# parsaeskandar/pangenome-index

Measured on AMD Instinct MI355X. Metric: find_mems reads/sec (150 bp batch), higher is better.
Workload: dtype u64

## Files before the change

### include/pgx.h

```cpp
#ifndef PGX_H
#define PGX_H

#include <stddef.h>
#include <stdint.h>

#ifdef __cplusplus
extern "C" {
#endif

#define PGX_ABI_VERSION 7

typedef enum {
    PGX_OK = 0,
    PGX_ERR_IO = 1,
    PGX_ERR_FORMAT = 2,
    PGX_ERR_UNSUPPORTED = 3,
    PGX_ERR_NO_DEVICE = 4,
    PGX_ERR_HIP = 5,
    PGX_ERR_ARG = 6,
    PGX_ERR_NOMEM = 7
} pgx_status;

#define PGX_MODE_COMPAT 0u
#define PGX_MODE_STRICT 1u
// ... 164 lines not shown
} pgx_timing;

#define PGX_KERNELS_FM 0x1u
#define PGX_KERNELS_FM_SEEDED 0x2u
#define PGX_KERNELS_FM_NARROW 0x4u
#define PGX_KERNELS_FM_KIND_SHIFT 3
#define PGX_KERNELS_FM_LDS 0x20u
#define PGX_KERNELS_FM_REDO 0x40u
#define PGX_KERNELS_PAIRS 0x100u
#define PGX_KERNELS_PAIRS_S64 0x200u
#define PGX_KERNELS_PAIRS_COOP 0x400u
#define PGX_KERNELS_PAIRS_PACKED 0x800u
#define PGX_KERNELS_PAIRS_WIDE 0x1000u
#define PGX_KERNELS_PAIRS_LCE 0x2000u
#define PGX_KERNELS_SIDE 0x10000u
#define PGX_KERNELS_HEAVY 0x20000u
#define PGX_KERNELS_FM_MASK 0x3Fu
#define PGX_KERNELS_PAIRS_MASK 0x3F00u
uint32_t pgx_kernel_variants(uint32_t *out, uint32_t cap);

pgx_status pgx_batch_create(pgx_index *h, int device, const uint8_t *reads, const uint64_t *offsets,
                            uint64_t n_reads, pgx_batch **out);
pgx_status pgx_host_alloc(size_t bytes, void **out);
void pgx_host_free(void *p);
pgx_status pgx_batch_upload(pgx_batch *b, const uint8_t *reads, const uint64_t *offsets, uint64_t n_reads);
pgx_status pgx_batch_upload_packed(pgx_batch *b, const uint32_t *packed, const uint64_t *offsets, uint64_t n_reads, const uint64_t *side_ids,
                                   const uint8_t *side_bytes, uint64_t n_side);
pgx_status pgx_pack_reads(const uint8_t *reads, const uint64_t *offsets, uint64_t n_reads, uint32_t threads, uint32_t *packed, uint64_t *side_ids,
                          uint64_t side_ids_cap, uint8_t *side_bytes, uint64_t side_bytes_cap, uint64_t *n_side, uint64_t *n_side_bytes);
#define PGX_READS_LINES 0u
// ... 76 lines not shown
```

### pangenome-index_amd/csrc/pgx_batch.hip

```cpp
#include <memory>
#include <string>
#include <thread>

#include "pgx_runtime_internal.hpp"

struct pgx_chunk { uint64_t r0, r1, slot_base, slots; };

struct pgx_batch {
    pgx_index *h = nullptr;
    pgx_device_image *dimg = nullptr;
    int device = 0;
    hipStream_t own = nullptr;
    hipStream_t side = nullptr;
    hipEvent_t ev_side[2] = {nullptr, nullptr};
    bool class_valid = false, class_ok = false;
    uint64_t side_reads_est = 0;
    uint64_t n_reads = 0, read_bytes = 0;
    HostBuf h_off[2];
    int h_off_cur = 0;
    const uint64_t *h_offsets() const { return h_off[h_off_cur].as<uint64_t>(); }
    std::vector<pgx_chunk> chunks;
    bool plan_valid = false, slot_off_valid = false;
    uint64_t slot_off_min_len = 0;
    uint64_t plan_min_len = 0, plan_budget = 0;
// ... 302 lines not shown
    return PGX_OK;
    PGX_GUARD_END
}


struct RunKnobs {
    bool spec;
    bool arena;
    bool has_arena_cap;
    uint64_t arena_cap;
    uint64_t budget_slots;
    bool narrow;
    bool force_redo;
    bool pairs;
    bool side;
    bool packed;
    int coop;
    bool lce;
    bool has_wg_per_cu;
    int wg_per_cu;
    uint32_t heavy_ext;
    bool has_side_heavy_ext;
    uint32_t side_heavy_ext;
    bool debug_counters;
    bool fm_stats;
};

static RunKnobs read_run_knobs() {
    auto is_set = [](const char *name) { return std::getenv(name) != nullptr; };
    auto not_zero = [](const char *name) { const char *e = std::getenv(name); return !(e && e[0] == '0'); };
    RunKnobs k{};
    k.spec = not_zero("PGX_SPEC");
    k.arena = not_zero("PGX_SLOT_ARENA");
    if (const char *e = std::getenv("PGX_SLOT_ARENA_CAP")) { k.has_arena_cap = true; k.arena_cap = std::strtoull(e, nullptr, 10); }
    if (const char *e = std::getenv("PGX_SLOT_BUDGET_MB")) k.budget_slots = std::max<uint64_t>(1, std::strtoull(e, nullptr, 10)) * (1ull << 20) / sizeof(pgx_mem);
    k.narrow = not_zero("PGX_FM_NARROW");
    k.force_redo = is_set("PGX_FM_NARROW_FORCE_REDO");
    k.pairs = not_zero("PGX_FM_PAIRS");
    k.side = !is_set("PGX_FM_NO_SIDE");
    k.packed = not_zero("PGX_FM_PACKED");
    k.coop = -1;
    if (const char *e = std::getenv("PGX_FM_COOP")) k.coop = e[0] == '1';
    k.lce = not_zero("PGX_FM_LCE");
    if (const char *e = std::getenv("PGX_FM_WG_PER_CU")) { k.has_wg_per_cu = true; k.wg_per_cu = std::atoi(e); }
    k.heavy_ext = PGX_FM_HEAVY_EXT;
    if (const char *e = std::getenv("PGX_FM_HEAVY_EXT")) k.heavy_ext = (uint32_t)std::strtoul(e, nullptr, 10);
    if (const char *e = std::getenv("PGX_FM_SIDE_HEAVY_EXT")) { k.has_side_heavy_ext = true; k.side_heavy_ext = (uint32_t)std::strtoul(e, nullptr, 10); }
    k.debug_counters = is_set("PGX_DEBUG_COUNTERS");
    k.fm_stats = is_set("PGX_FM_STATS");
    return k;
}

static const void *find_mems_entry(bool in_lds, uint32_t kind, bool narrow, bool seeded) {
    using K = const void *;
// ... 15 lines not shown
static uint32_t find_mems_bits(bool in_lds, uint32_t kind, bool narrow, bool seeded) {
    return PGX_KERNELS_FM | (seeded ? PGX_KERNELS_FM_SEEDED : 0u) | (narrow ? PGX_KERNELS_FM_NARROW : 0u) | (kind << PGX_KERNELS_FM_KIND_SHIFT) | (in_lds ? PGX_KERNELS_FM_LDS : 0u);
}

static const void *find_mems_variant(bool in_lds, uint32_t kind, bool narrow, bool seeded, uint32_t &bits) {
    if (kind == 0) seeded = false;
    const void *f = find_mems_entry(in_lds, kind, narrow, seeded);
    if (!f) throw Error(PGX_ERR_UNSUPPORTED, "pgx_batch_run: no find_mems kernel for this image");
    bits = find_mems_bits(in_lds, kind, narrow, seeded);
    return f;
}

static const void *find_mems_pairs_entry(bool wide, bool packed, bool coop, bool s64, bool lce) {
    using K = const void *;
    static const K plain[2][2] = {
        {(K)pgx_find_mems_pairs_kernel<true, false, false, false, false, false>, (K)pgx_find_mems_pairs_kernel<true, false, false, false, true, false>},
        {(K)pgx_find_mems_pairs_kernel<true, true, false, false, false, false>, (K)pgx_find_mems_pairs_kernel<true, true, false, false, true, false>}};
    static const K pack[2][2][2] = {
        {{(K)pgx_find_mems_pairs_kernel<true, false, true, false, false, false>, (K)pgx_find_mems_pairs_kernel<true, false, true, false, true, false>},
         {(K)pgx_find_mems_pairs_kernel<true, false, true, true, false, false>, (K)pgx_find_mems_pairs_kernel<true, false, true, true, true, false>}},
        {{(K)pgx_find_mems_pairs_kernel<true, true, true, false, false, false>, (K)pgx_find_mems_pairs_kernel<true, true, true, false, true, false>},
         {(K)pgx_find_mems_pairs_kernel<true, true, true, true, false, false>, (K)pgx_find_mems_pairs_kernel<true, true, true, true, true, false>}}};
    static const K with_lce[2] = {(K)pgx_find_mems_pairs_kernel<true, false, true, false, false, true>, (K)pgx_find_mems_pairs_kernel<true, false, true, false, true, true>};
    if (lce) return (wide || !packed || coop) ? nullptr : with_lce[s64];
    if (!packed) return coop ? nullptr : plain[wide][s64];
    return pack[wide][coop][s64];
}

static uint32_t find_mems_pairs_bits(bool wide, bool packed, bool coop, bool s64, bool lce) {
    return PGX_KERNELS_PAIRS | (s64 ? PGX_KERNELS_PAIRS_S64 : 0u) | (coop ? PGX_KERNELS_PAIRS_COOP : 0u) | (packed ? PGX_KERNELS_PAIRS_PACKED : 0u) |
           (wide ? PGX_KERNELS_PAIRS_WIDE : 0u) | (lce ? PGX_KERNELS_PAIRS_LCE : 0u);
}

static const void *find_mems_pairs_variant(bool wide, bool packed, bool coop, bool s64, bool lce, uint32_t &bits) {
    const void *f = find_mems_pairs_entry(wide, packed, coop, s64, lce);
    if (!f && lce) throw Error(PGX_ERR_UNSUPPORTED, "pgx_batch_run: no LCE pairs kernel for this image");
    if (!f) throw Error(PGX_ERR_UNSUPPORTED, "pgx_batch_run: no cooperative pairs kernel without the packed reads");
    bits = find_mems_pairs_bits(wide, packed, coop, s64, lce);
    return f;
}

// ... 11 lines not shown
    }
    return n;
}

struct RunCtx {
    pgx_batch *b;
    hipStream_t s;
    RunKnobs k;
    PgxDevImage img;
    uint64_t n, min_len, min_occ;
    bool want_tags;
    unsigned long long *ctr = nullptr;
    bool spec = false, arena_on = false;
    uint64_t cm_cap = 0;
    const void *kfn = nullptr, *kfn_wide = nullptr, *kfn_pairs = nullptr;
    uint32_t kfn_bits = 0, kfn_pairs_bits = 0;
    size_t pairs_lds = 0;
    int cus = 0;
    bool fresh_work = false, fresh_mark = false;
    uint64_t n_ext = 0;
    float ms_fm = 0, ms_cp = 0, ms_main = 0;
};

struct FmArgs {
    PgxDevImage img;
    const uint8_t *reads;
    const uint64_t *off, *slot_off;
    uint64_t n, min_len, min_occ, base, first;
    pgx_mem *slots;
    uint32_t *cnt;
// ... 62 lines not shown
    }
    uint64_t max_chunk_reads = 1;
    for (auto &c : b->chunks) max_chunk_reads = std::max(max_chunk_reads, c.r1 - c.r0);
    b->ovf_base.ensure(max_chunk_reads * 4);
}

static void choose_kernels(RunCtx &r) {
    pgx_batch *b = r.b;
    const PgxDevImage &img = r.img;
    const bool in_lds = b->dimg->lds_bytes != 0;
    const bool seeded = img.seed_k != 0 && r.min_len >= img.seed_k;
    r.kfn = r.kfn_wide = find_mems_variant(in_lds, img.dense, false, seeded, r.kfn_bits);
    bool c_fits = true;
    for (int i = 0; i < 8; i++) c_fits = c_fits && !(b->h->img.consts.C[i] >> 32);
    if (img.dense && img.dense != 3 && img.n < (1ull << 30) && c_fits && r.k.narrow) r.kfn = find_mems_variant(in_lds, img.dense, true, seeded, r.kfn_bits);
    r.kfn_pairs = nullptr;
    if (img.pairs && seeded && !(r.n >> 32) && b->read_bytes < (1ull << 35) && r.k.pairs)
        r.kfn_pairs = find_mems_pairs_variant(img.wide != 0, false, false, img.pairs_stride == PGX_PAIRS_STRIDE64, false, r.kfn_pairs_bits);
    r.pairs_lds = img.wide ? (size_t)img.n_sbp * 192 : 0;
    HIPCHECK(hipDeviceGetAttribute(&r.cus, hipDeviceAttributeMultiprocessorCount, b->device));
}

static void classify_reads(RunCtx &r, uint64_t cn) {
    pgx_batch *b = r.b;
    hipStream_t s = r.s;
    r.fresh_work = true;
    const uint64_t cap = std::max<uint64_t>(cn, 1024);
    b->read_flags.ensure(((cn + 3) & ~3ull) + 4);
    b->side_list.ensure((cn ? cn : 1) * sizeof(pgx_heavy_item));
    b->side_count.ensure(16);
    b->scan_tmp.ensure(cap * 8);
    b->scan_tmp.scan_epoch = 0;
    b->packed.ensure(((b->read_bytes + 15) / 16 + 64) * 4);
// ... 17 lines not shown
}

static void launch_side(RunCtx &r, FmArgs &a, const void *kf, unsigned grid) {
    pgx_batch *b = r.b;
    HIPCHECK(hipEventRecord(b->ev_side[0], r.s));
    HIPCHECK(hipStreamWaitEvent(b->side, b->ev_side[0], 0));
    const pgx_heavy_item *s_list = b->side_list.as<pgx_heavy_item>();
    const unsigned long long *s_count = b->side_count.as<unsigned long long>();
    unsigned long long *s_cur = r.ctr + PGX_CTR_SIDE_CURSOR;
    uint32_t s_hext = r.k.heavy_ext ? std::min<uint32_t>(r.k.heavy_ext, PGX_FM_SIDE_HEAVY_EXT) : 0u;
    if (r.k.has_side_heavy_ext) s_hext = r.k.side_heavy_ext;
    void *sargs[] = {&a.img, &a.reads, &a.off, &a.n, &a.min_len, &a.min_occ, &a.slot_off, &a.slots, &a.cnt, &a.next, &s_cur, &a.first, &a.base,
                     &s_hext, &a.hcap, &a.hlist, &a.hcount, &s_list, &s_count, &a.ovf, &a.ovf_cap};
    const uint64_t cus = (uint64_t)r.cus;
    const unsigned side_wgs = (unsigned)std::min<uint64_t>(4 * cus, std::max<uint64_t>(cus, b->side_reads_est / (2ull * PGX_FM_THREADS) + 1));
    HIPCHECK(hipLaunchKernel(kf, dim3(std::min<unsigned>(grid, side_wgs)), dim3(PGX_FM_THREADS), sargs, b->dimg->lds_bytes, b->side));
    b->timing.kernels |= r.kfn_bits | PGX_KERNELS_SIDE | (kf != r.kfn ? PGX_KERNELS_FM_REDO : 0u);
    HIPCHECK(hipEventRecord(b->ev_side[1], b->side));
}

static void launch_pairs(RunCtx &r, FmArgs &a, const uint8_t *skip, uint64_t cn, unsigned grid) {
    pgx_batch *b = r.b;
    const PgxDevImage &img = r.img;
    const void *kp = r.kfn_pairs;
    uint32_t kp_bits = r.kfn_pairs_bits;
    size_t plds = r.pairs_lds;
    const uint32_t *a_packed = nullptr;
    uint32_t a_pkw = 0;
    const uint32_t pkw = (uint32_t)((15 + b->max_read_len + 15) >> 4) + 1u;
    if (skip && pkw <= 24 && r.k.packed) {
        const bool coop = r.k.coop >= 0 ? r.k.coop != 0 : b->h->img.pairs.size() > (3ull << 30);
// ... 203 lines not shown
    pgx_batch *b = r.b;
    hipStream_t s = r.s;
    b->n_mems = b->n_positions = b->n_ext = b->n_tag_overflow = 0;
    std::memset(&b->timing, 0, sizeof b->timing);
    r.fresh_work = r.fresh_mark = false;
    r.n_ext = 0;
    r.ms_fm = r.ms_cp = r.ms_main = 0;
    b->counters.ensure(PGX_CTR_ALL * 8);
    HIPCHECK(hipMemsetAsync(b->counters.p, 0, PGX_CTR_ALL * 8, s));
    r.ctr = b->counters.as<unsigned long long>();

    record(b, 0, s);
    plan_slots(r);
    const std::vector<pgx_chunk> &chunks = b->chunks;
    r.arena_on = r.k.arena && !force_worst;
    r.kfn = r.kfn_wide = r.kfn_pairs = nullptr;
    r.cus = 0;
    if (r.n) choose_kernels(r);
    if (r.k.heavy_ext) {
        b->heavy_list.ensure((size_t)PGX_FM_HEAVY_CAP * sizeof(pgx_heavy_item));
        b->heavy_scratch.ensure((size_t)PGX_FM_HEAVY_GRID * PGX_FM_HEAVY_MAXLEN * sizeof(PgxHeavyResult));
    }
    r.spec = may_speculate && chunks.size() == 1 && b->shape_valid && b->shape_reads == r.n && b->shape_min_len == r.min_len && b->shape_min_occ == r.min_occ &&
             b->shape_tags == r.want_tags && (!r.want_tags || (b->tw.have_last && b->tw.last_largest <= PGX_SORT_WG_LDS_CAP)) && r.k.spec && !r.k.force_redo;
    r.cm_cap = with_slack(b->last_mems);
    uint64_t mem_base = 0;
    for (size_t ci = 0; ci < chunks.size(); ci++) {
        record(b, 1, s);
        uint64_t ovf_cap = 0;
        const uint64_t cm = find_mems_chunk(r, ci, ovf_cap);
        compact_chunk(r, chunks[ci], cm, mem_base, ovf_cap);
// ... 402 lines not shown
```

### pangenome-index_amd/csrc/pgx_device.h

```cpp
#pragma once

#include <hip/hip_runtime.h>
#include <stdint.h>

#include "../../include/pgx.h"
#include "pgx_image.h"

enum PgxCounterSlot {
    PGX_CTR_EXT = 0,
    PGX_CTR_TAG_OVERFLOW = 1,
    PGX_CTR_CURSOR = 5,
    PGX_CTR_HEAVY = 8,
    PGX_CTR_OVF32 = 9,
    PGX_CTR_MEMS = 10,
    PGX_CTR_REDO = 11,
    PGX_CTR_REDO_CURSOR = 12,
    PGX_CTR_SIDE_CURSOR = 13,
    PGX_CTR_OVF_TOP = 14,
    PGX_CTR_OVF_ABORT = 15,
    PGX_CTR_TAG0 = 16,
    PGX_CTR_ABORT = 30,
    PGX_CTR_PAIRS_LINES = 32,
    PGX_CTR_PAIRS_SEEDS = 33,
    PGX_CTR_FM_LINES = 34,
// ... 77 lines not shown
#define PGX_FM_HEAVY_GRID 64u
template <bool LDS_IMAGE>
__global__ void pgx_find_mems_heavy_kernel(PgxDevImage img, const uint8_t *reads, const uint64_t *offsets, uint64_t min_len, uint64_t min_occ,
                                           const uint64_t *slot_off, uint64_t slot_base, pgx_mem *slots, uint32_t *mem_count,
                                           unsigned long long *n_ext_total, const pgx_heavy_item *heavy_list,
                                           const unsigned long long *heavy_count, uint32_t heavy_cap, PgxHeavyResult *scratch, uint64_t chunk_first,
                                           uint64_t chunk_reads, uint32_t *ovf_base, uint64_t ovf_cap);

__global__ void pgx_seed_build_kernel(PgxDevImage img, const uint4 *src, uint4 *dst, uint32_t level, uint64_t n_dst, uint64_t limit, int end_table);
template <bool LDS_IMAGE, int DENSE, bool NARROW, bool SEED>
__global__ void pgx_find_mems_kernel(PgxDevImage img, const uint8_t *reads, const uint64_t *offsets, uint64_t n_reads,
                                     uint64_t min_len, uint64_t min_occ, const uint64_t *slot_off, pgx_mem *slots,
                                     uint32_t *mem_count, unsigned long long *n_ext_total, unsigned long long *cursor, uint64_t first_read,
                                     uint64_t slot_base, uint32_t heavy_ext, uint32_t heavy_cap, pgx_heavy_item *heavy_list, unsigned long long *heavy_count,
                                     const pgx_heavy_item *rid_list, const unsigned long long *rid_count, uint32_t *ovf_base, uint64_t ovf_cap);
template <bool SEED, bool WIDE, bool PACKED, bool COOP, bool S64, bool LCE>
__global__ void pgx_find_mems_pairs_kernel(PgxDevImage img, const uint8_t *reads, const uint64_t *offsets, uint64_t n_reads,
                                           uint64_t min_len, uint64_t min_occ, const uint64_t *slot_off, pgx_mem *slots,
                                           uint32_t *mem_count, unsigned long long *n_ext_total, unsigned long long *cursor, uint64_t first_read,
                                           uint64_t slot_base, uint32_t heavy_ext, uint32_t heavy_cap, pgx_heavy_item *heavy_list, unsigned long long *heavy_count,
                                           const uint8_t *skip, const uint32_t *packed, uint32_t pk_words,
                                           uint32_t *ovf_base, uint64_t ovf_cap);
__global__ void pgx_bad_chunks_kernel(const uint8_t *reads, uint64_t n_bytes, uint64_t *chunks, unsigned long long *count, uint64_t cap, uint32_t *packed);
__global__ void pgx_unpack_reads_kernel(const uint32_t *packed, uint64_t n_chunks, uint8_t *reads);
__global__ void pgx_side_reads_kernel(uint8_t *reads, const uint64_t *offsets, const uint64_t *side_ids, const uint64_t *side_off, const uint8_t *side_bytes, uint64_t n_side,
                                      uint8_t *flags, pgx_heavy_item *list, unsigned long long *count);
__global__ void pgx_classify_reads_kernel(const uint8_t *reads, const uint64_t *offsets, uint64_t n_reads, const uint64_t *chunks, const unsigned long long *n_chunks,
                                          uint64_t cap, uint32_t *flag_words, pgx_heavy_item *list, unsigned long long *count);
__global__ void pgx_first_ext_kernel(PgxDevImage img, uint4 *out);
__global__ void pgx_rank_kernel(PgxDevImage img, const uint64_t *pos, uint64_t n, int true_codes, uint64_t *out);
template <bool LOOP, bool MULHI> __global__ void pgx_rank_probe_kernel(PgxDevImage img, const uint64_t *pos, uint64_t n, uint64_t *out);
// ... 145 lines not shown
```

### pangenome-index_amd/csrc/pgx_kernels.hip

```cpp
#include <hip/hip_runtime.h>
#include <stdint.h>

#include <type_traits>

#include "pgx_device.h"

template <bool LDS_IMAGE>
__device__ __forceinline__ uint32_t pgx_find_block(const PgxDevImage &img, const uint64_t *__restrict__ lds_dir,
                                                   const uint16_t *__restrict__ lds_blow, uint64_t pos) {
    const uint64_t di = pos >> img.dir_shift;
    const uint64_t e = LDS_IMAGE ? lds_dir[di] : img.dir[di];
    const uint32_t lowp = (uint32_t)pos & ((1u << img.dir_shift) - 1u);
    uint32_t lo = (uint32_t)e;
    const uint32_t cnt = (uint32_t)(e >> 32) & 0xFFu;
    if (cnt <= 2) {
        const uint32_t l0 = (uint32_t)(e >> 40) & 0xFFFu, l1 = (uint32_t)(e >> 52);
        return lo - 1u + ((cnt >= 1 && l0 <= lowp) ? 1u : 0u) + ((cnt >= 2 && l1 <= lowp) ? 1u : 0u);
    }
    uint32_t hi = cnt < 255 ? lo + cnt : (uint32_t)(LDS_IMAGE ? lds_dir[di + 1] : img.dir[di + 1]);
    while (lo < hi) {
        const uint32_t mid = (lo + hi) >> 1;
        const uint32_t v = LDS_IMAGE ? lds_blow[mid] : img.blow[mid];
        if (v <= lowp) lo = mid + 1; else hi = mid;
    }
// ... 856 lines not shown
    if (k >= n_side) return;
    const uint64_t rid = side_ids[k], dst = offsets[rid], len = offsets[rid + 1] - dst, src = side_off[k];
    for (uint64_t i = lane; i < len; i += 64) reads[dst + i] = side_bytes[src + i];
    if (lane == 0) {
        flags[rid] = 1;
        pgx_heavy_item it;
        it.rid = rid; it.x = 0; it.nm = 0;
        list[k] = it;
        if (k == 0) *count = n_side;
    }
}

__device__ __forceinline__ uint32_t pgx_window_byte(uint64_t w0, uint64_t w1, uint64_t a) {
    return (uint32_t)(((a & 8ull) ? w1 : w0) >> (8u * (uint32_t)(a & 7ull))) & 0xFFu;
}
template <bool SEED, bool WIDE, bool PACKED, bool COOP, bool S64, bool LCE>
#ifndef PGX_LCE_WAVES
#define PGX_LCE_WAVES PGX_FM_WAVES_PER_SIMD
#endif
__global__ void __launch_bounds__(PGX_FM_THREADS, LCE ? PGX_LCE_WAVES : ((PACKED && !WIDE && !COOP) ? PGX_PAIRS_PACKED_WAVES : PGX_FM_WAVES_PER_SIMD))
pgx_find_mems_pairs_kernel(PgxDevImage img, const uint8_t *__restrict__ reads, const uint64_t *__restrict__ offsets,
                           uint64_t n_reads, uint64_t min_len, uint64_t min_occ, const uint64_t *__restrict__ slot_off,
                           pgx_mem *__restrict__ slots, uint32_t *__restrict__ mem_count, unsigned long long *__restrict__ n_ext_total,
                           unsigned long long *__restrict__ cursor, uint64_t first_read, uint64_t slot_base, uint32_t heavy_ext, uint32_t heavy_cap,
                           pgx_heavy_item *__restrict__ heavy_list, unsigned long long *__restrict__ heavy_count, const uint8_t *__restrict__ skip,
                           const uint32_t *__restrict__ packed, uint32_t pk_words, uint32_t *__restrict__ ovf_base, uint64_t ovf_cap) {
    typedef typename std::conditional<WIDE, uint64_t, uint32_t>::type pos_t;
    __shared__ uint32_t s_ext[512];
    __shared__ pos_t s_C[8];
    __shared__ pos_t s_t2[32];
    __shared__ uint4 s_fe[PACKED ? 16 : 512];
    extern __shared__ __align__(16) unsigned char pgx_dyn_lds[];
    static_assert(!COOP || PACKED, "the cooperative loads come with the packed reads");
    static_assert(!LCE || (PACKED && !WIDE && !COOP), "the text comparison reads the packed reads and 32-bit suffix array entries");
    constexpr uint32_t SYMS = PGX_PAIRS_SYMS, STRIDE = S64 ? PGX_PAIRS_STRIDE64 : PGX_PAIRS_SYMS;
    uint32_t *s_rd = reinterpret_cast<uint32_t *>(pgx_dyn_lds);
    const uint32_t rd_stride = blockDim.x;
    uint4 *s_stage = reinterpret_cast<uint4 *>(pgx_dyn_lds + (size_t)pk_words * PGX_FM_THREADS * 4) + (size_t)(threadIdx.x >> 6) * 512;
    uint64_t *s_pb = reinterpret_cast<uint64_t *>(pgx_dyn_lds + (size_t)pk_words * PGX_FM_THREADS * 4 + (COOP ? (size_t)(PGX_FM_THREADS / 64) * 8192 : 0));
    uint4 *s_sa4 = reinterpret_cast<uint4 *>(pgx_dyn_lds + (size_t)pk_words * PGX_FM_THREADS * 4);
    uint32_t *s_sae = reinterpret_cast<uint32_t *>(s_sa4 + PGX_FM_THREADS);
    uint32_t *s_lcp = s_sae + PGX_FM_THREADS;
    for (uint32_t i = threadIdx.x; i < 512; i += blockDim.x) s_ext[i] = img.consts->ext_tab[i];
    if (threadIdx.x < 8) s_C[threadIdx.x] = (pos_t)img.consts->C[threadIdx.x];
    if (threadIdx.x < 32) s_t2[threadIdx.x] = (pos_t)img.consts->pair_t2w[threadIdx.x];
    if (WIDE) for (uint32_t i = threadIdx.x; i < img.n_sbp * 24u; i += blockDim.x) s_pb[i] = img.pbase[i];
    if (PACKED) { if (threadIdx.x < 9) s_fe[threadIdx.x] = img.first_ext[threadIdx.x == 4 ? 0u : (threadIdx.x > 4 ? 256u : 0u) + ((0x47544341u >> (8u * ((threadIdx.x > 4 ? threadIdx.x - 5u : threadIdx.x) & 3u))) & 0xFFu)]; }
    else for (uint32_t i = threadIdx.x; i < 512; i += blockDim.x) s_fe[i] = img.first_ext[i];
    __syncthreads();
// ... 88 lines not shown
        restart = more ? restart : 1u;
    };

    for (;;) {
        __builtin_amdgcn_s_setprio(3);
        unsigned long long idle = __ballot(ph == 0);
        if (LCE && idle && (uint32_t)__popcll(idle) < img.refill_min && __popcll(idle) != 64) idle = 0ull;
#ifdef PGX_FM_STATS
        const unsigned long long st_r0 = __builtin_readcyclecounter();
        if (idle) st_refills++;
#endif
        while (idle) {
            if (rnext == rend) {
                if (exhausted) break;
                unsigned long long got = 0;
                if (lane == 0) got = first_read + atomicAdd(cursor, 32ull);
                got = ((unsigned long long)(uint32_t)__builtin_amdgcn_readfirstlane((int)(uint32_t)(got >> 32)) << 32) |
                      (uint32_t)__builtin_amdgcn_readfirstlane((int)(uint32_t)got);
                if (got >= n_reads) { exhausted = true; break; }
                rnext = got;
                rend = got + 32ull < n_reads ? got + 32ull : n_reads;
            }
            const uint64_t avail = rend - rnext;
            const uint32_t rank = (uint32_t)__popcll(idle & ((1ull << lane) - 1ull));
            if (ph == 0 && (uint64_t)rank < avail) {
                rid = (uint32_t)(rnext + rank);
                const uint8_t *skp = skip ? skip + rid : reinterpret_cast<const uint8_t *>(offsets);
                const uint32_t skv = (uint32_t)*skp;
                const uint64_t o0 = offsets[rid], o1 = offsets[rid + 1];
                const uint32_t sk = skip ? skv : 0u;
                base = o0;
                len = (int32_t)(o1 - o0);
                if (sk) ph = -1;
                else {
                    if (PACKED) {
                        const uint32_t *src = packed + (base >> 4);
                        const uint32_t nw = ((uint32_t)(base & 15ull) + (uint32_t)len + 15u) >> 4;
#pragma unroll 1
                        for (uint32_t w0 = 0; w0 < nw; w0 += PGX_PK_GROUP) {
                            uint32_t t[PGX_PK_GROUP];
#pragma unroll
                            for (uint32_t i = 0; i < PGX_PK_GROUP; i++) t[i] = src[w0 + i < nw ? w0 + i : nw - 1u];
#pragma unroll
                            for (uint32_t i = 0; i < PGX_PK_GROUP; i++) if (w0 + i < nw) s_rd[(w0 + i) * rd_stride + threadIdx.x] = t[i];
                        }
                    }
                    x = 0; nm = 0;
                    next0 = next;
                    begin();
                    if (ph == 0) ph = -1;
                }
            }
            const uint32_t want = (uint32_t)__popcll(idle);
            rnext += (uint64_t)want < avail ? (uint64_t)want : avail;
            idle = __ballot(ph == 0);
        }
#ifdef PGX_FM_STATS
        asm volatile("s_waitcnt vmcnt(0) lgkmcnt(0)" ::: "memory");
        st_t_refill += __builtin_readcyclecounter() - st_r0;
#endif
        if (ph == -1) ph = 0;
        if (!__any(ph > 0)) {
// ... 216 lines not shown
#ifdef PGX_FM_STATS
                const unsigned long long st_l0 = __builtin_readcyclecounter();
#endif
                const uint4 *bp = img.pairs + (size_t)(bfirst + pend) * 8;
                if (LCE && PGX_LCE_ASM_LOADS) {
                    const uint4 *rp = bp + t1;
                    asm volatile("global_load_dwordx4 %0, %3, off\n\tglobal_load_dwordx4 %1, %4, off offset:64\n\tglobal_load_dwordx4 %2, %4, off offset:80"
                                 : "+v"(row), "+v"(hs), "+v"(d0) : "v"(rp), "v"(bp) : "memory");
                    d1 = ld4(bp + 6); d2 = ld4(bp + 7);
                } else {
                    row = ld4(bp + t1); hs = ld4(bp + 4); d0 = ld4(bp + 5); d1 = ld4(bp + 6); d2 = ld4(bp + 7);
                }
#ifdef PGX_EXP_LOAD6
                { const uint4 xx = bp[(t1 + 1u) & 3u]; asm volatile("" ::"v"(xx.x), "v"(xx.y), "v"(xx.z), "v"(xx.w)); }
#endif
                __builtin_amdgcn_s_setprio(0);
#ifdef PGX_FM_STATS
                asm volatile("s_waitcnt vmcnt(0)" : "+v"(row), "+v"(hs), "+v"(d0), "+v"(d1), "+v"(d2) :: "memory");
                st_t_line += __builtin_readcyclecounter() - st_l0;
#endif
            }
            const uint32_t i0 = (t1 & 1u) ? 0u : 0xFFFFFFFFu, i1 = (t1 & 2u) ? 0u : 0xFFFFFFFFu, j0 = (t2 & 1u) ? 0u : 0xFFFFFFFFu, j1 = (t2 & 2u) ? 0u : 0xFFFFFFFFu;
            const uint32_t ua = t1 < 2u ? 0xFFFFFFFFu : 0u, va = t1 == 0u ? 0xFFFFFFFFu : 0u, wa = (t1 & 1u) ? 0u : 0xFFFFFFFFu;
            const uint32_t ub = t2 < 2u ? 0xFFFFFFFFu : 0u, vb = t2 == 0u ? 0xFFFFFFFFu : 0u, wb = (t2 & 1u) ? 0u : 0xFFFFFFFFu;
            if (LCE && !COOP && PGX_LCE_ASM_LOADS) asm volatile("s_waitcnt vmcnt(0)" : "+v"(row), "+v"(hs), "+v"(d0) :: "memory");
            const bool flagged = (hs.x >> 31) != 0u;
            const uint32_t pts = (t1 == 0u ? hs.x : (t1 == 1u ? hs.y : (t1 == 2u ? hs.z : hs.w))) & 0x00FFFFFFu;
            const uint32_t PX[3] = {d0.x, d0.y, d0.z}, PY[3] = {d0.w, d1.x, d1.y}, PU[3] = {d1.z, d1.w, d2.x}, PV[3] = {d2.y, d2.z, d2.w};
            uint32_t e1p = 0, e2p = 0, e1r = 0, g1r = 0, e2r = 0, g2r = 0;
#pragma unroll
            for (int h = 0; h < 3; h++) {
// ... 67 lines not shown
                    for (int it = 0; it < 2; it++) {
                        const uint64_t q = it ? q1 : q0;
                        uint64_t a, bq;
                        if (WIDE) pgx_dense2w_rank(img, q, PGX_EXT_CV(e1), PGX_EXT_M(e1), a, bq);
                        else if (img.dense == 1) {
                            const PgxDenseBlk db = pgx_dense_load<false>(img, nullptr, q);
                            pgx_dense_rank(db, q, PGX_EXT_CV(e1), PGX_EXT_M(e1), a, bq);
                        } else pgx_dense2_rank(img, (uint32_t)q, PGX_EXT_CV(e1), PGX_EXT_M(e1), a, bq);
                        A1 = a; B1 = bq;
                        if (!it) { A0 = a; B0 = bq; }
                    }
                    const uint64_t dB = B1 - B0;
                    {
                        const unsigned long long here = __ballot(true);
                        if (lane == (int)__ffsll((long long)here) - 1) {
                            atomicAdd(n_ext_total + PGX_CTR_REDO, (unsigned long long)__popcll(here));
                            atomicAdd(n_ext_total + PGX_CTR_PAIRS_LINES, 2ull * (unsigned long long)__popcll(here));
                        }
                    }
                    const bool none = PGX_EXT_KILL(e1) || A0 >= A1;
                    s1 = none ? (pos_t)0 : (pos_t)(A1 - A0);
                    k1 = (pos_t)A0 + s_C[PGX_EXT_V(e1)];
                    q1v = kq + (pos_t)dB;
                }
                if (fr) { const uint4 f = s_fe[PACKED ? (at_end ? 4u : ((byte >> 1) & 3u)) : byte]; k1 = ent_k(f); q1v = ent_q(f); s1 = ent_s(f); }
                const bool small1 = s1 == 0u || s1 < mo || mo_huge;
                const uint32_t sdepth = se.w >> 24;
                const pos_t se_s = ent_s(se);
                const bool seed_alive = SEED && seed_lane && se_s != 0u && se_s >= mo && !mo_huge;
                const bool seed_dead = SEED && seed_lane && se_s == 0u && sdepth != PGX_SEED_UNUSABLE && min_occ <= 1;
                const bool do2 = (fr ? (at_end && rem2 && have2 && !seed_alive && !seed_dead) : (two && !bail && !cont1)) && !small1;
                pos_t s2 = (pos_t)c2, k2 = r2 + s_C[PGX_EXT_V(e2)] + s_t2[8u * t1 + cv2], q2v = q1v + (pos_t)w2;
// ... 109 lines not shown
                    j += (int32_t)lce_best;
                    lce_st = 0u;
                    em_now = true;
                }
            }
        }
        if (em_now) emit();
        if (restart) begin();
        if (FUSE) prefetch();
    }
    unsigned long long tot = next;
#pragma unroll
    for (int off = 32; off > 0; off >>= 1) tot += __shfl_down(tot, off, 64);
    if (lane == 0 && tot) atomicAdd(n_ext_total + PGX_CTR_EXT, tot);
    ln_two += (unsigned long long)__popcll(__ballot(did2 != 0u));
    if (lane == 0 && ln_blk) { atomicAdd(n_ext_total + PGX_CTR_PAIRS_LINES, ln_blk); atomicAdd(n_ext_total + PGX_CTR_PAIRS_SEEDS, ln_seed); atomicAdd(n_ext_total + PGX_CTR_PAIRS_TWO, ln_two); }
#ifdef PGX_FM_STATS
#pragma unroll
    for (int off = 32; off > 0; off >>= 1) st_wait += __shfl_down(st_wait, off, 64);
    if (lane == 0) { atomicAdd(n_ext_total + PGX_CTR_ST_PAIR_T_REFILL, st_t_refill); atomicAdd(n_ext_total + PGX_CTR_ST_PAIR_T_TOTAL, __builtin_readcyclecounter() - st_t0); atomicAdd(n_ext_total + PGX_CTR_ST_PAIR_REFILLS, st_refills);
                     atomicAdd(n_ext_total + PGX_CTR_ST_PAIR_T_SEED, st_t_seed); atomicAdd(n_ext_total + PGX_CTR_ST_PAIR_T_LINE, st_t_line); }
    if (lane == 0) { atomicAdd(n_ext_total + PGX_CTR_ST_PAIR_TRIPS, st_trips); atomicAdd(n_ext_total + PGX_CTR_ST_PAIR_LIVE, st_live); atomicAdd(n_ext_total + PGX_CTR_ST_PAIR_WAIT, st_wait); atomicAdd(n_ext_total + PGX_CTR_ST_PAIR_FRESH, st_fresh); }
#endif
}
#define PGX_PAIRS_INSTANTIATE(...)                                                                                                                \
    template __global__ void pgx_find_mems_pairs_kernel<__VA_ARGS__>(PgxDevImage, const uint8_t *, const uint64_t *, uint64_t, uint64_t, uint64_t, const uint64_t *, \
                                                                     pgx_mem *, uint32_t *, unsigned long long *, unsigned long long *, uint64_t, uint64_t, uint32_t, \
                                                                     uint32_t, pgx_heavy_item *, unsigned long long *, const uint8_t *, const uint32_t *, uint32_t,  \
                                                                     uint32_t *, uint64_t);
PGX_PAIRS_INSTANTIATE(true, false, false, false, false, false)
PGX_PAIRS_INSTANTIATE(true, true, false, false, false, false)
PGX_PAIRS_INSTANTIATE(true, false, true, false, false, false)
PGX_PAIRS_INSTANTIATE(true, true, true, false, false, false)
PGX_PAIRS_INSTANTIATE(true, false, true, true, false, false)
PGX_PAIRS_INSTANTIATE(true, true, true, true, false, false)
PGX_PAIRS_INSTANTIATE(true, false, false, false, true, false)
PGX_PAIRS_INSTANTIATE(true, true, false, false, true, false)
PGX_PAIRS_INSTANTIATE(true, false, true, false, true, false)
PGX_PAIRS_INSTANTIATE(true, true, true, false, true, false)
PGX_PAIRS_INSTANTIATE(true, false, true, true, true, false)
PGX_PAIRS_INSTANTIATE(true, true, true, true, true, false)
PGX_PAIRS_INSTANTIATE(true, false, true, false, false, true)
PGX_PAIRS_INSTANTIATE(true, false, true, false, true, true)

__global__ void __launch_bounds__(256) pgx_first_ext_kernel(PgxDevImage img, uint4 *__restrict__ out) {
    __shared__ uint32_t s_ext[512];
    __shared__ uint64_t s_C[8];
    pgx_stage_tables<false>(img, s_ext, s_C, nullptr, nullptr, nullptr);
    uint64_t k = 0, kp = 0, s = img.n;
    pgx_extend<false>(img, nullptr, nullptr, nullptr, s_ext, s_C, k, kp, s, threadIdx.x, false);
    auto pack = [](uint64_t k_, uint64_t q_, uint64_t s_) {
        return make_uint4((uint32_t)k_, (uint32_t)q_, (uint32_t)s_, (uint32_t)((k_ >> 32) & 0xFFu) | ((uint32_t)((q_ >> 32) & 0xFFu) << 8) | ((uint32_t)((s_ >> 32) & 0xFFu) << 16));
    };
    out[threadIdx.x] = pack(k, kp, s);
    k = 0; kp = 0; s = img.n;
    pgx_extend<false>(img, nullptr, nullptr, nullptr, s_ext, s_C, k, kp, s, 0u, false);
    if (s) pgx_extend<false>(img, nullptr, nullptr, nullptr, s_ext, s_C, k, kp, s, threadIdx.x, false);
    out[256 + threadIdx.x] = pack(k, kp, s);
// ... 496 lines not shown
```

### pangenome-index_amd/pgx_ffi.py

```python
import ctypes as C
import os
import subprocess

import numpy as np

PKG_DIR = os.path.dirname(os.path.abspath(__file__))
ROOT = os.path.dirname(PKG_DIR)
LIB_PATH = os.environ.get("PGX_LIB") or os.path.join(PKG_DIR, "libpgx.so")

OK, ERR_IO, ERR_FORMAT, ERR_UNSUPPORTED, ERR_NO_DEVICE, ERR_HIP, ERR_ARG, ERR_NOMEM = range(8)
MODE_COMPAT, MODE_STRICT = 0, 1
MODE_IMAGE_RL, MODE_IMAGE_DENSE, MODE_IMAGE_DENSE2, MODE_IMAGE_PAIRS = 0x100, 0x200, 0x400, 0x800
MODE_IMAGE_WIDE = 0x1000
IMAGE_RL, IMAGE_DENSE, IMAGE_DENSE2 = 0, 1, 2
TAGS_AUTO, TAGS_BYTECODE, TAGS_COMPACT = 0, 1, 2
RUN_TAGS, RUN_TIMING = 1, 2
READS_LINES, READS_FASTA, READS_FASTQ = 0, 1, 2

MEM_DTYPE = np.dtype([("start", "<u8"), ("end", "<u8"), ("bwt_start", "<u8"), ("size", "<i8")])
BIINT_DTYPE = np.dtype([("forward", "<u8"), ("reverse", "<u8"), ("size", "<i8")])

u64, u32, p = C.c_uint64, C.c_uint32, C.c_void_p


# ... 38 lines not shown


class Timing(C.Structure):
    _fields_ = [
        ("ms_find_mems", C.c_float), ("ms_compact", C.c_float), ("ms_tag_locate", C.c_float),
        ("ms_tag_gather", C.c_float), ("ms_tag_sort", C.c_float), ("ms_total", C.c_float),
        ("find_mems_launches", u32), ("heavy_reads", u32), ("pairs_reads", u32), ("pairs_other_steps", u32),
        ("ms_find_mems_main", C.c_float), ("seed_depth", u32),
        ("main_lines", u64), ("main_seed_loads", u64), ("other_lines", u64), ("other_seed_loads", u64), ("two_step_trips", u64),
        ("ms_per_upload", C.c_float), ("kernels", u32),
    ]


KERNELS_FM, KERNELS_FM_SEEDED, KERNELS_FM_NARROW, KERNELS_FM_KIND_SHIFT, KERNELS_FM_LDS, KERNELS_FM_REDO = 0x1, 0x2, 0x4, 3, 0x20, 0x40
KERNELS_PAIRS, KERNELS_PAIRS_S64, KERNELS_PAIRS_COOP, KERNELS_PAIRS_PACKED, KERNELS_PAIRS_WIDE, KERNELS_PAIRS_LCE = 0x100, 0x200, 0x400, 0x800, 0x1000, 0x2000
KERNELS_SIDE, KERNELS_HEAVY = 0x10000, 0x20000
KERNELS_FM_MASK, KERNELS_PAIRS_MASK = 0x3F, 0x3F00


def kernel_variants():
    n = lib().pgx_kernel_variants(None, 0)
    out = np.zeros(n, dtype=np.uint32)
    assert lib().pgx_kernel_variants(out.ctypes.data, n) == n
    return [int(v) for v in out]


def _u64_array(ptr, n):
    if n == 0 or not ptr:
        return np.zeros(0, dtype=np.uint64)
    return np.ctypeslib.as_array(ptr, shape=(n,)).copy()

# ... 592 lines not shown
```

Measured before the change: 1.124 billion.

## Run side-read list through the two-step pairs kernel instead of one-step FM kernel

Adds a LIST template variant of the pairs kernel that pulls read ids, start positions and match counts from the side (non-ACGT) read list. It launches this variant on the side stream in place of the one-step find_mems kernel, enabled by default through PGX_FM_SIDE_TWO_STEP. The aim is to give side reads the faster two-symbol-per-step extension. The cost is more kernel instantiations, different LDS sizing for the side launch, and reliance on byte windows for reads holding unusual symbols.

```diff
diff --git a/include/pgx.h b/include/pgx.h
--- a/include/pgx.h
+++ b/include/pgx.h
@@ -202,6 +202,7 @@
 #define PGX_KERNELS_PAIRS_WIDE 0x1000u
 #define PGX_KERNELS_PAIRS_LCE 0x2000u
 #define PGX_KERNELS_SIDE 0x10000u
+#define PGX_KERNELS_SIDE_ONE_STEP 0x40000u
 #define PGX_KERNELS_HEAVY 0x20000u
 #define PGX_KERNELS_FM_MASK 0x3Fu
 #define PGX_KERNELS_PAIRS_MASK 0x3F00u
diff --git a/pangenome-index_amd/csrc/pgx_batch.hip b/pangenome-index_amd/csrc/pgx_batch.hip
--- a/pangenome-index_amd/csrc/pgx_batch.hip
+++ b/pangenome-index_amd/csrc/pgx_batch.hip
@@ -340,6 +340,7 @@
     bool force_redo;
     bool pairs;
     bool side;
+    bool side_two_step;
     bool packed;
     int coop;
     bool lce;
@@ -364,6 +365,7 @@
     k.force_redo = is_set("PGX_FM_NARROW_FORCE_REDO");
     k.pairs = not_zero("PGX_FM_PAIRS");
     k.side = !is_set("PGX_FM_NO_SIDE");
+    k.side_two_step = not_zero("PGX_FM_SIDE_TWO_STEP");
     k.packed = not_zero("PGX_FM_PACKED");
     k.coop = -1;
     if (const char *e = std::getenv("PGX_FM_COOP")) k.coop = e[0] == '1';
@@ -409,17 +411,25 @@
 static const void *find_mems_pairs_entry(bool wide, bool packed, bool coop, bool s64, bool lce) {
     using K = const void *;
     static const K plain[2][2] = {
-        {(K)pgx_find_mems_pairs_kernel<true, false, false, false, false, false>, (K)pgx_find_mems_pairs_kernel<true, false, false, false, true, false>},
-        {(K)pgx_find_mems_pairs_kernel<true, true, false, false, false, false>, (K)pgx_find_mems_pairs_kernel<true, true, false, false, true, false>}};
+        {(K)pgx_find_mems_pairs_kernel<true, false, false, false, false, false, false>, (K)pgx_find_mems_pairs_kernel<true, false, false, false, true, false, false>},
+        {(K)pgx_find_mems_pairs_kernel<true, true, false, false, false, false, false>, (K)pgx_find_mems_pairs_kernel<true, true, false, false, true, false, false>}};
     static const K pack[2][2][2] = {
-        {{(K)pgx_find_mems_pairs_kernel<true, false, true, false, false, false>, (K)pgx_find_mems_pairs_kernel<true, false, true, false, true, false>},
-         {(K)pgx_find_mems_pairs_kernel<true, false, true, true, false, false>, (K)pgx_find_mems_pairs_kernel<true, false, true, true, true, false>}},
-        {{(K)pgx_find_mems_pairs_kernel<true, true, true, false, false, false>, (K)pgx_find_mems_pairs_kernel<true, true, true, false, true, false>},
-         {(K)pgx_find_mems_pairs_kernel<true, true, true, true, false, false>, (K)pgx_find_mems_pairs_kernel<true, true, true, true, true, false>}}};
-    static const K with_lce[2] = {(K)pgx_find_mems_pairs_kernel<true, false, true, false, false, true>, (K)pgx_find_mems_pairs_kernel<true, false, true, false, true, true>};
+        {{(K)pgx_find_mems_pairs_kernel<true, false, true, false, false, false, false>, (K)pgx_find_mems_pairs_kernel<true, false, true, false, true, false, false>},
+         {(K)pgx_find_mems_pairs_kernel<true, false, true, true, false, false, false>, (K)pgx_find_mems_pairs_kernel<true, false, true, true, true, false, false>}},
+        {{(K)pgx_find_mems_pairs_kernel<true, true, true, false, false, false, false>, (K)pgx_find_mems_pairs_kernel<true, true, true, false, true, false, false>},
+         {(K)pgx_find_mems_pairs_kernel<true, true, true, true, false, false, false>, (K)pgx_find_mems_pairs_kernel<true, true, true, true, true, false, false>}}};
+    static const K with_lce[2] = {(K)pgx_find_mems_pairs_kernel<true, false, true, false, false, true, false>, (K)pgx_find_mems_pairs_kernel<true, false, true, false, true, true, false>};
     if (lce) return (wide || !packed || coop) ? nullptr : with_lce[s64];
     if (!packed) return coop ? nullptr : plain[wide][s64];
     return pack[wide][coop][s64];
+}
+
+static const void *find_mems_pairs_list_entry(bool wide, bool s64) {
+    using K = const void *;
+    static const K tab[2][2] = {
+        {(K)pgx_find_mems_pairs_kernel<true, false, false, false, false, false, true>, (K)pgx_find_mems_pairs_kernel<true, false, false, false, true, false, true>},
+        {(K)pgx_find_mems_pairs_kernel<true, true, false, false, false, false, true>, (K)pgx_find_mems_pairs_kernel<true, true, false, false, true, false, true>}};
+    return tab[wide][s64];
 }
 
 static uint32_t find_mems_pairs_bits(bool wide, bool packed, bool coop, bool s64, bool lce) {
@@ -461,6 +471,7 @@
     bool spec = false, arena_on = false;
     uint64_t cm_cap = 0;
     const void *kfn = nullptr, *kfn_wide = nullptr, *kfn_pairs = nullptr;
+    const void *kfn_side = nullptr;
     uint32_t kfn_bits = 0, kfn_pairs_bits = 0;
     size_t pairs_lds = 0;
     int cus = 0;
@@ -553,9 +564,10 @@
     bool c_fits = true;
     for (int i = 0; i < 8; i++) c_fits = c_fits && !(b->h->img.consts.C[i] >> 32);
     if (img.dense && img.dense != 3 && img.n < (1ull << 30) && c_fits && r.k.narrow) r.kfn = find_mems_variant(in_lds, img.dense, true, seeded, r.kfn_bits);
-    r.kfn_pairs = nullptr;
+    r.kfn_pairs = r.kfn_side = nullptr;
     if (img.pairs && seeded && !(r.n >> 32) && b->read_bytes < (1ull << 35) && r.k.pairs)
         r.kfn_pairs = find_mems_pairs_variant(img.wide != 0, false, false, img.pairs_stride == PGX_PAIRS_STRIDE64, false, r.kfn_pairs_bits);
+    if (r.kfn_pairs && r.k.side_two_step) r.kfn_side = find_mems_pairs_list_entry(img.wide != 0, img.pairs_stride == PGX_PAIRS_STRIDE64);
     r.pairs_lds = img.wide ? (size_t)img.n_sbp * 192 : 0;
     HIPCHECK(hipDeviceGetAttribute(&r.cus, hipDeviceAttributeMultiprocessorCount, b->device));
 }
@@ -603,7 +615,17 @@
                      &s_hext, &a.hcap, &a.hlist, &a.hcount, &s_list, &s_count, &a.ovf, &a.ovf_cap};
     const uint64_t cus = (uint64_t)r.cus;
     const unsigned side_wgs = (unsigned)std::min<uint64_t>(4 * cus, std::max<uint64_t>(cus, b->side_reads_est / (2ull * PGX_FM_THREADS) + 1));
-    HIPCHECK(hipLaunchKernel(kf, dim3(std::min<unsigned>(grid, side_wgs)), dim3(PGX_FM_THREADS), sargs, b->dimg->lds_bytes, b->side));
+    if (r.kfn_side) {
+        const uint8_t *l_list = reinterpret_cast<const uint8_t *>(s_list);
+        const uint32_t *l_count = reinterpret_cast<const uint32_t *>(s_count);
+        uint32_t l_pkw = 0;
+        void *largs[] = {&a.img, &a.reads, &a.off, &a.n, &a.min_len, &a.min_occ, &a.slot_off, &a.slots, &a.cnt, &a.next, &s_cur, &a.first, &a.base,
+                         &s_hext, &a.hcap, &a.hlist, &a.hcount, &l_list, &l_count, &l_pkw, &a.ovf, &a.ovf_cap};
+        HIPCHECK(hipLaunchKernel(r.kfn_side, dim3(std::min<unsigned>(grid, side_wgs)), dim3(PGX_FM_THREADS), largs, r.pairs_lds, b->side));
+    } else {
+        HIPCHECK(hipLaunchKernel(kf, dim3(std::min<unsigned>(grid, side_wgs)), dim3(PGX_FM_THREADS), sargs, b->dimg->lds_bytes, b->side));
+        b->timing.kernels |= PGX_KERNELS_SIDE_ONE_STEP;
+    }
     b->timing.kernels |= r.kfn_bits | PGX_KERNELS_SIDE | (kf != r.kfn ? PGX_KERNELS_FM_REDO : 0u);
     HIPCHECK(hipEventRecord(b->ev_side[1], b->side));
 }
@@ -837,7 +859,7 @@
     plan_slots(r);
     const std::vector<pgx_chunk> &chunks = b->chunks;
     r.arena_on = r.k.arena && !force_worst;
-    r.kfn = r.kfn_wide = r.kfn_pairs = nullptr;
+    r.kfn = r.kfn_wide = r.kfn_pairs = r.kfn_side = nullptr;
     r.cus = 0;
     if (r.n) choose_kernels(r);
     if (r.k.heavy_ext) {
diff --git a/pangenome-index_amd/csrc/pgx_device.h b/pangenome-index_amd/csrc/pgx_device.h
--- a/pangenome-index_amd/csrc/pgx_device.h
+++ b/pangenome-index_amd/csrc/pgx_device.h
@@ -115,7 +115,7 @@
                                      uint32_t *mem_count, unsigned long long *n_ext_total, unsigned long long *cursor, uint64_t first_read,
                                      uint64_t slot_base, uint32_t heavy_ext, uint32_t heavy_cap, pgx_heavy_item *heavy_list, unsigned long long *heavy_count,
                                      const pgx_heavy_item *rid_list, const unsigned long long *rid_count, uint32_t *ovf_base, uint64_t ovf_cap);
-template <bool SEED, bool WIDE, bool PACKED, bool COOP, bool S64, bool LCE>
+template <bool SEED, bool WIDE, bool PACKED, bool COOP, bool S64, bool LCE, bool LIST>
 __global__ void pgx_find_mems_pairs_kernel(PgxDevImage img, const uint8_t *reads, const uint64_t *offsets, uint64_t n_reads,
                                            uint64_t min_len, uint64_t min_occ, const uint64_t *slot_off, pgx_mem *slots,
                                            uint32_t *mem_count, unsigned long long *n_ext_total, unsigned long long *cursor, uint64_t first_read,
diff --git a/pangenome-index_amd/csrc/pgx_kernels.hip b/pangenome-index_amd/csrc/pgx_kernels.hip
--- a/pangenome-index_amd/csrc/pgx_kernels.hip
+++ b/pangenome-index_amd/csrc/pgx_kernels.hip
@@ -894,7 +894,7 @@
 __device__ __forceinline__ uint32_t pgx_window_byte(uint64_t w0, uint64_t w1, uint64_t a) {
     return (uint32_t)(((a & 8ull) ? w1 : w0) >> (8u * (uint32_t)(a & 7ull))) & 0xFFu;
 }
-template <bool SEED, bool WIDE, bool PACKED, bool COOP, bool S64, bool LCE>
+template <bool SEED, bool WIDE, bool PACKED, bool COOP, bool S64, bool LCE, bool LIST>
 #ifndef PGX_LCE_WAVES
 #define PGX_LCE_WAVES PGX_FM_WAVES_PER_SIMD
 #endif
@@ -913,6 +913,10 @@
     extern __shared__ __align__(16) unsigned char pgx_dyn_lds[];
     static_assert(!COOP || PACKED, "the cooperative loads come with the packed reads");
     static_assert(!LCE || (PACKED && !WIDE && !COOP), "the text comparison reads the packed reads and 32-bit suffix array entries");
+    static_assert(!LIST || (!PACKED && !COOP && !LCE), "the listed reads hold bytes outside A C G T: byte windows only");
+    const pgx_heavy_item *const rid_list = LIST ? reinterpret_cast<const pgx_heavy_item *>(skip) : nullptr;
+    const uint64_t q_first = LIST ? 0ull : first_read;
+    const uint64_t q_end = LIST ? (uint64_t)*reinterpret_cast<const unsigned long long *>(packed) : n_reads;
     constexpr uint32_t SYMS = PGX_PAIRS_SYMS, STRIDE = S64 ? PGX_PAIRS_STRIDE64 : PGX_PAIRS_SYMS;
     uint32_t *s_rd = reinterpret_cast<uint32_t *>(pgx_dyn_lds);
     const uint32_t rd_stride = blockDim.x;
@@ -1031,21 +1035,23 @@
             if (rnext == rend) {
                 if (exhausted) break;
                 unsigned long long got = 0;
-                if (lane == 0) got = first_read + atomicAdd(cursor, 32ull);
+                if (lane == 0) got = q_first + atomicAdd(cursor, 32ull);
                 got = ((unsigned long long)(uint32_t)__builtin_amdgcn_readfirstlane((int)(uint32_t)(got >> 32)) << 32) |
                       (uint32_t)__builtin_amdgcn_readfirstlane((int)(uint32_t)got);
-                if (got >= n_reads) { exhausted = true; break; }
+                if (got >= q_end) { exhausted = true; break; }
                 rnext = got;
-                rend = got + 32ull < n_reads ? got + 32ull : n_reads;
+                rend = got + 32ull < q_end ? got + 32ull : q_end;
             }
             const uint64_t avail = rend - rnext;
             const uint32_t rank = (uint32_t)__popcll(idle & ((1ull << lane) - 1ull));
             if (ph == 0 && (uint64_t)rank < avail) {
                 rid = (uint32_t)(rnext + rank);
-                const uint8_t *skp = skip ? skip + rid : reinterpret_cast<const uint8_t *>(offsets);
+                uint32_t x0 = 0u, nm0 = 0u;
+                if (LIST) { const pgx_heavy_item it = rid_list[rnext + rank]; rid = (uint32_t)it.rid; x0 = it.x; nm0 = it.nm; }
+                const uint8_t *skp = (skip && !LIST) ? skip + rid : reinterpret_cast<const uint8_t *>(offsets);
                 const uint32_t skv = (uint32_t)*skp;
                 const uint64_t o0 = offsets[rid], o1 = offsets[rid + 1];
-                const uint32_t sk = skip ? skv : 0u;
+                const uint32_t sk = (skip && !LIST) ? skv : 0u;
                 base = o0;
                 len = (int32_t)(o1 - o0);
                 if (sk) ph = -1;
@@ -1062,7 +1068,7 @@
                             for (uint32_t i = 0; i < PGX_PK_GROUP; i++) if (w0 + i < nw) s_rd[(w0 + i) * rd_stride + threadIdx.x] = t[i];
                         }
                     }
-                    x = 0; nm = 0;
+                    x = (int32_t)x0; nm = nm0;
                     next0 = next;
                     begin();
                     if (ph == 0) ph = -1;
@@ -1309,7 +1315,7 @@
 #ifdef PGX_EXP_LOAD6
                 { const uint4 xx = bp[(t1 + 1u) & 3u]; asm volatile("" ::"v"(xx.x), "v"(xx.y), "v"(xx.z), "v"(xx.w)); }
 #endif
-                __builtin_amdgcn_s_setprio(0);
+                if (!LIST) __builtin_amdgcn_s_setprio(0);
 #ifdef PGX_FM_STATS
                 asm volatile("s_waitcnt vmcnt(0)" : "+v"(row), "+v"(hs), "+v"(d0), "+v"(d1), "+v"(d2) :: "memory");
                 st_t_line += __builtin_readcyclecounter() - st_l0;
@@ -1407,8 +1413,8 @@
                     {
                         const unsigned long long here = __ballot(true);
                         if (lane == (int)__ffsll((long long)here) - 1) {
-                            atomicAdd(n_ext_total + PGX_CTR_REDO, (unsigned long long)__popcll(here));
-                            atomicAdd(n_ext_total + PGX_CTR_PAIRS_LINES, 2ull * (unsigned long long)__popcll(here));
+                            if (!LIST) atomicAdd(n_ext_total + PGX_CTR_REDO, (unsigned long long)__popcll(here));
+                            atomicAdd(n_ext_total + (LIST ? PGX_CTR_FM_LINES : PGX_CTR_PAIRS_LINES), 2ull * (unsigned long long)__popcll(here));
                         }
                     }
                     const bool none = PGX_EXT_KILL(e1) || A0 >= A1;
@@ -1548,8 +1554,13 @@
     for (int off = 32; off > 0; off >>= 1) tot += __shfl_down(tot, off, 64);
     if (lane == 0 && tot) atomicAdd(n_ext_total + PGX_CTR_EXT, tot);
     ln_two += (unsigned long long)__popcll(__ballot(did2 != 0u));
-    if (lane == 0 && ln_blk) { atomicAdd(n_ext_total + PGX_CTR_PAIRS_LINES, ln_blk); atomicAdd(n_ext_total + PGX_CTR_PAIRS_SEEDS, ln_seed); atomicAdd(n_ext_total + PGX_CTR_PAIRS_TWO, ln_two); }
+    if (LIST) { if (lane == 0 && (ln_blk | ln_seed)) { atomicAdd(n_ext_total + PGX_CTR_FM_LINES, ln_blk); atomicAdd(n_ext_total + PGX_CTR_FM_SEEDS, ln_seed); } }
+    else if (lane == 0 && ln_blk) { atomicAdd(n_ext_total + PGX_CTR_PAIRS_LINES, ln_blk); atomicAdd(n_ext_total + PGX_CTR_PAIRS_SEEDS, ln_seed); atomicAdd(n_ext_total + PGX_CTR_PAIRS_TWO, ln_two); }
 #ifdef PGX_FM_STATS
+    if (LIST) {
+        if (lane == 0) { atomicAdd(n_ext_total + PGX_CTR_ST_TRIPS, st_trips); atomicAdd(n_ext_total + PGX_CTR_ST_LIVE, st_live); atomicMax(n_ext_total + PGX_CTR_ST_LONGEST, st_trips); }
+        return;
+    }
 #pragma unroll
     for (int off = 32; off > 0; off >>= 1) st_wait += __shfl_down(st_wait, off, 64);
     if (lane == 0) { atomicAdd(n_ext_total + PGX_CTR_ST_PAIR_T_REFILL, st_t_refill); atomicAdd(n_ext_total + PGX_CTR_ST_PAIR_T_TOTAL, __builtin_readcyclecounter() - st_t0); atomicAdd(n_ext_total + PGX_CTR_ST_PAIR_REFILLS, st_refills);
@@ -1562,20 +1573,24 @@
                                                                      pgx_mem *, uint32_t *, unsigned long long *, unsigned long long *, uint64_t, uint64_t, uint32_t, \
                                                                      uint32_t, pgx_heavy_item *, unsigned long long *, const uint8_t *, const uint32_t *, uint32_t,  \
                                                                      uint32_t *, uint64_t);
-PGX_PAIRS_INSTANTIATE(true, false, false, false, false, false)
-PGX_PAIRS_INSTANTIATE(true, true, false, false, false, false)
-PGX_PAIRS_INSTANTIATE(true, false, true, false, false, false)
-PGX_PAIRS_INSTANTIATE(true, true, true, false, false, false)
-PGX_PAIRS_INSTANTIATE(true, false, true, true, false, false)
-PGX_PAIRS_INSTANTIATE(true, true, true, true, false, false)
-PGX_PAIRS_INSTANTIATE(true, false, false, false, true, false)
-PGX_PAIRS_INSTANTIATE(true, true, false, false, true, false)
-PGX_PAIRS_INSTANTIATE(true, false, true, false, true, false)
-PGX_PAIRS_INSTANTIATE(true, true, true, false, true, false)
-PGX_PAIRS_INSTANTIATE(true, false, true, true, true, false)
-PGX_PAIRS_INSTANTIATE(true, true, true, true, true, false)
-PGX_PAIRS_INSTANTIATE(true, false, true, false, false, true)
-PGX_PAIRS_INSTANTIATE(true, false, true, false, true, true)
+PGX_PAIRS_INSTANTIATE(true, false, false, false, false, false, false)
+PGX_PAIRS_INSTANTIATE(true, true, false, false, false, false, false)
+PGX_PAIRS_INSTANTIATE(true, false, true, false, false, false, false)
+PGX_PAIRS_INSTANTIATE(true, true, true, false, false, false, false)
+PGX_PAIRS_INSTANTIATE(true, false, true, true, false, false, false)
+PGX_PAIRS_INSTANTIATE(true, true, true, true, false, false, false)
+PGX_PAIRS_INSTANTIATE(true, false, false, false, true, false, false)
+PGX_PAIRS_INSTANTIATE(true, true, false, false, true, false, false)
+PGX_PAIRS_INSTANTIATE(true, false, true, false, true, false, false)
+PGX_PAIRS_INSTANTIATE(true, true, true, false, true, false, false)
+PGX_PAIRS_INSTANTIATE(true, false, true, true, true, false, false)
+PGX_PAIRS_INSTANTIATE(true, true, true, true, true, false, false)
+PGX_PAIRS_INSTANTIATE(true, false, true, false, false, true, false)
+PGX_PAIRS_INSTANTIATE(true, false, true, false, true, true, false)
+PGX_PAIRS_INSTANTIATE(true, false, false, false, false, false, true)
+PGX_PAIRS_INSTANTIATE(true, true, false, false, false, false, true)
+PGX_PAIRS_INSTANTIATE(true, false, false, false, true, false, true)
+PGX_PAIRS_INSTANTIATE(true, true, false, false, true, false, true)
 
 __global__ void __launch_bounds__(256) pgx_first_ext_kernel(PgxDevImage img, uint4 *__restrict__ out) {
     __shared__ uint32_t s_ext[512];
diff --git a/pangenome-index_amd/pgx_ffi.py b/pangenome-index_amd/pgx_ffi.py
--- a/pangenome-index_amd/pgx_ffi.py
+++ b/pangenome-index_amd/pgx_ffi.py
@@ -76,7 +76,7 @@
 
 KERNELS_FM, KERNELS_FM_SEEDED, KERNELS_FM_NARROW, KERNELS_FM_KIND_SHIFT, KERNELS_FM_LDS, KERNELS_FM_REDO = 0x1, 0x2, 0x4, 3, 0x20, 0x40
 KERNELS_PAIRS, KERNELS_PAIRS_S64, KERNELS_PAIRS_COOP, KERNELS_PAIRS_PACKED, KERNELS_PAIRS_WIDE, KERNELS_PAIRS_LCE = 0x100, 0x200, 0x400, 0x800, 0x1000, 0x2000
-KERNELS_SIDE, KERNELS_HEAVY = 0x10000, 0x20000
+KERNELS_SIDE, KERNELS_HEAVY, KERNELS_SIDE_ONE_STEP = 0x10000, 0x20000, 0x40000
 KERNELS_FM_MASK, KERNELS_PAIRS_MASK = 0x3F, 0x3F00
 
 
```

After: 928.2 million. -17.4%, worse.
